# rishikksh20/FastSpeech2

Measured on AMD Instinct MI355X. Metric: mel-frames/sec, higher is better.
Workload: dtype bf16x3 (FFN conv: f16 x f16 + block-scaled e4m3 cross terms; the decoder's: block-scaled e2m1 cross terms, one E8M0 scale per 16-channel block on both operands); 1 GPU; c3: batch=64 LJSpeech-shape; default.yaml dims, free-running, random-init weights (seed 0), duration bias calibrated to 7.87 frames/phoneme; precision=mix_mx4, utterances=64, phonemes=4528, parallelism=single GPU, launch=eager, device-driven layout (no host sync), overlap_encoder=False, streams=3

## Files before the change

fastspeech2_amd/csrc/elementwise.h:

```cpp
#pragma once
#include "common.h"

namespace fs2 {

__global__ void build_row_meta(const int* start, const int* len, int B, int rpad, int* row_pos, int* row_seq) {
    const int row = blockIdx.x * blockDim.x + threadIdx.x;
    if (row >= rpad) return;
    int lo = 0, hi = B;
    while (lo < hi) {
        const int mid = (lo + hi) >> 1;
        if (start[mid] <= row) lo = mid + 1; else hi = mid;
    }
    const int b = lo - 1;
    int pos = -1, seq = -1;
    if (b >= 0 && row - start[b] < len[b]) { pos = row - start[b]; seq = b; }
    row_pos[row] = pos;
    row_seq[row] = seq;
}

__global__ __launch_bounds__(1024) void frame_layout_dev(const int* olens, int B, int compat, int masked, int row_cap, int work_cap,
                                                         int lmax_cap, int pe_rows, int* start, int* len, int* klen, int* vlen,
                                                         int* rank_tmp, int* woff_tmp, int* pcum, int2* work, int* dims, int* status = nullptr, int gap = 8) {
    constexpr int kStage = 4096;
    __shared__ int s_len[kStage], s_vlen[kStage], s_order[kStage];
// ... 195 lines not shown
        }
        if (lane == 63) wsum[wave] = x;
        __syncthreads();
        int off = carry_s;
        for (int w = 0; w < wave; ++w) off += wsum[w];
        if (t < T) cum[(size_t)b * Tmax + t] = off + x;
        __syncthreads();
        if (tid == 255) carry_s = off + x;
        __syncthreads();
    }
    if (tid == 0) {
        const int tt = bad_s ? -1 : (ones ? T : total);
        if (olens) olens[b] = tt;
        if (olens32) olens32[b] = tt;
    }
}

__global__ __launch_bounds__(256) void lr_expand(const float* hs, int D, const int* tok_start, const int* ilen,
                                                 const int* cum, int Tmax, const int* row_pos, const int* row_seq,
                                                 int uniform_len, const int* vlen, int R, float* out,
                                                 int* index_rows, void* planes = nullptr) {
    const int row = __builtin_amdgcn_readfirstlane(blockIdx.x * 4 + (threadIdx.x >> 6));
    const int lane = threadIdx.x & 63;
    if (row >= R) return;
    int b, j;
    if (row_seq) { b = row_seq[row]; j = row_pos[row]; } else { b = row / uniform_len; j = row - b * uniform_len; }
    float* dst = out + (size_t)row * D;
    int idx = -1;
    if (b >= 0 && j < vlen[b]) {
        const int* c = cum + (size_t)b * Tmax;
// ... 59 lines not shown
    const float* te = Te + (size_t)qe * D;
    const float* tp = Tp + (size_t)qp * D;
    for (int c = lane * 4; c < D; c += 256) {
        float4 v = *reinterpret_cast<const float4*>(dst + c);
        const float4 a = *reinterpret_cast<const float4*>(tp + c);
        const float4 g = *reinterpret_cast<const float4*>(te + c);
        v.x = (v.x + a.x) + g.x;
        v.y = (v.y + a.y) + g.y;
        v.z = (v.z + a.z) + g.z;
        v.w = (v.w + a.w) + g.w;
        *reinterpret_cast<float4*>(dst + c) = v;
        if (planes) store_planes4(planes, row, D / 32, c, f32x4{v.x, v.y, v.z, v.w});
    }
}

template <typename T>
__global__ void unpack_rows(const T* src, int W, const int* start, const int* limit, int B, int Lout, T* dst, T fill) {
    const int64_t i = (int64_t)blockIdx.x * blockDim.x + threadIdx.x;
    const int64_t total = (int64_t)B * Lout * W;
    if (i >= total) return;
    const int w = (int)(i % W);
    const int64_t bj = i / W;
    const int j = (int)(bj % Lout), b = (int)(bj / Lout);
    dst[i] = (j < limit[b]) ? src[(size_t)(start[b] + j) * W + w] : fill;
}

__global__ void unpack_rows4(const float* src, int W4, const int* start, const int* limit, int B, int Lout, float* dst, const int* ovf = nullptr) {
    const int64_t i = (int64_t)blockIdx.x * blockDim.x + threadIdx.x;
    if (i >= (int64_t)B * Lout * W4) return;
    const int w = (int)(i % W4);
// ... 90 lines not shown
```

fastspeech2_amd/csrc/fs2_runtime.hip:

```cpp
#include <hip/hip_runtime.h>
#include <dlfcn.h>

#include <algorithm>
#include <cmath>
#include <cstdarg>
#include <cstdio>
#include <cstring>
#include <fstream>
#include <iterator>
#include <map>
#include <string>
#include <type_traits>
#include <vector>

#include "../../include/fs2.h"
#include "attn_bf16.h"
#include "attn_w32.h"
#include "attn_f32.h"
#include "common.h"
#include "elementwise.h"
#include "gemm_bf16.h"
#include "gemm_plan.h"
#include "gemm_planes.h"
#include "gemm_row4.h"
// ... 7 lines not shown
namespace {

std::string g_create_error;

struct Gemm {
    float* w = nullptr;
    void* wb = nullptr;
    void* wf = nullptr;
    void* wm = nullptr;
    int kw = 0;
    void* wm4 = nullptr;
    unsigned char* ws4 = nullptr;
    float* bias = nullptr;
    int N = 0, C = 0, Cpad = 0, ktaps = 1;
};
struct Layer {
    Gemm qkv, out, w1, w2;
    Gemm cat_x, cat_a;
    float *ln1g = nullptr, *ln1b = nullptr, *ln2g = nullptr, *ln2b = nullptr;
    int ka = 0;
    int kh = 0;
};
struct Predictor {
    std::vector<Gemm> conv;
    std::vector<float*> lng, lnb;
    float *lin_w = nullptr, *lin_b = nullptr;
};
struct FusedPredictors {
    bool ok = false;
    Gemm c0, c1;
// ... 87 lines not shown
        if (sf.gcount() > 0) sh.update(blk.data(), (size_t)sf.gcount());
    }
    return sh.hex16() == want;
}
bool audit_clean() {
    static const bool ok = audit_clean_of_this_binary();
    return ok;
}

Options& opts() {
    static Options o = [] {
        Options x;
        x.bm = env_int("FS2_BM", -1); x.row8 = env_int("FS2_ROW8", -1); x.qkv8 = env_int("FS2_QKV8", -1);
        x.nosplitk = env_int("FS2_NOSPLITK", 0) != 0; x.f32_rows = env_int("FS2_F32_ROWS", 0) != 0; x.mt8 = env_int("FS2_MT8", -1); x.qkv_split = env_int("FS2_QKV_SPLIT", -1); x.op_att_planes = env_int("FS2_OP_ATT_PLANES", 0); x.fuse_var = env_int("FS2_FUSE_VAR", 1); x.bal = env_int("FS2_BAL", 0); x.w32 = env_int("FS2_ATTN_W32", -1);
        x.row4 = env_int("FS2_ROW4", -1); x.mt4 = env_int("FS2_MT4", -1); x.ffn2_mx = env_int("FS2_FFN2_MX", 1); x.qkv4 = env_int("FS2_QKV4", -1); x.post_mx = env_int("FS2_POST_MX", 1);
        if (!audit_clean()) {
            x.w32 = 0; x.row4 = 0; x.qkv4 = 0;
            fprintf(stderr, "libfs2_hip: no clean ISA-audit record of this binary (libfs2_hip.audit.json next to it): attn_w32 and gemm_row4_bf16 are switched "
                            "off, attn_bf16 / gemm_row8_bf16 run instead; rebuild with `python -c 'import __graft_entry__ as g; g.build()'`\n");
        }
        return x;
    }();
    return o;
}

inline int padded_head_dim(int dk) { return dk <= 64 ? 64 : (dk <= 128 ? 128 : (dk <= 192 ? 192 : (dk <= 256 ? 256 : 0))); }
inline int att_width(int D, int heads) { return heads * padded_head_dim(D / heads); }

inline int base_precision(int p) { return (p == FS2_PREC_MIX_F16X2 || p == FS2_PREC_MIX_F16X1 || p == FS2_PREC_MIX_MX || p == FS2_PREC_MIX_MX4) ? FS2_PREC_BF16X3 : p; }
constexpr int kFfnMx = 9;
// ... 66 lines not shown
struct ProfRec { std::string name; hipEvent_t e0, e1; double flops, bytes; };

}

struct fs2_handle {
    fs2_config cfg;
    std::string err;
    bool loaded = false;
    std::vector<void*> allocs;
    float* enc_embed = nullptr;
    Stack enc, dec;
    Predictor dur, energy, pitch;
    FusedPredictors var2;
    float *ebins = nullptr, *pbins = nullptr, *Te = nullptr, *Tp = nullptr;
    Gemm dec_in; float *dec_in_lng = nullptr, *dec_in_lnb = nullptr;
    Gemm feat;
    std::vector<Gemm> post;
    bool encoded = false;
    HostLayout tok;
    DevLayout dtok;
    float* enc_final = nullptr;
    int* cum = nullptr;
    int* o32 = nullptr;
    int enc_B = 0, enc_Tmax = 0, enc_compat = 0;
    long enc_ntok = 0;
    float* kp = nullptr; size_t kp_cap = 0;
    int cur_regime = 0;
    int* counters = nullptr;
    int* cur_status = nullptr;
    int gap = kGap;
    void* enc_ws = nullptr;
    std::vector<void*> graph_pinned;
    bool prof = false;
    std::string prof_filter;
    std::vector<ProfRec> recs;
};
// ... 595 lines not shown
        a.relu_pre = 1; a.ln_g = p.lng[l]; a.ln_b = p.lnb[l]; a.ln_eps = 1e-12f;
        if (last) { a.dot_w = p.lin_w; a.dot_b = p.lin_b; a.dot_out = out_rows; }
        a.scratch = out;
        a.Xp = Xp; a.xp_scratch = xps;
        if (xps && !last) { a.Yp = xps; a.yp_chunks = round_up(p.conv[l].N, 32) / 32; }
        if (xps && !last) Xp = xps; else Xp = nullptr;
        snprintf(nm, sizeof nm, "%s.conv%d", tag, (int)l);
        int rc = launch_gemm(h, s, nm, a, prec);
        if (rc) return rc;
        in = out; ld = p.conv[l].N;
    }
    return FS2_OK;
}

int run_predictors_fused(fs2_handle* h, hipStream_t s, const FusedPredictors& v, const float* X, int ldx, int R, const int* row_pos, const int* Rp,
                         const void* Xp, void* xps, float* vp, float* vs, float* e_rows, float* p_rows, int prec) {
    const int chans = v.c0.N / 2;
    int rc;
    const bool row8 = row_regime(h->cur_regime ? h->cur_regime : R, opts().row8);
    if (row8 && (chans == 256 || chans == 384)) {
        const Predictor* ps[2] = {&h->energy, &h->pitch};
        for (int g = 0; g < 2; ++g) {
            GemmArgs a = gemm_args(ps[g]->conv[0], X, ldx, R, row_pos, nullptr, chans);
            a.Rp = Rp; a.relu_pre = 1; a.ln_g = ps[g]->lng[0]; a.ln_b = ps[g]->lnb[0]; a.ln_eps = 1e-12f;
            a.Xp = Xp; a.xp_scratch = xps; a.Yp = vp; a.yp_chunks = v.c0.N / 32; a.yp_col_off = g * chans; a.scratch = vs;
            if ((rc = launch_gemm(h, s, g ? "pitch.conv0" : "energy.conv0", a, prec))) return rc;
        }
    } else {
        GemmArgs a = gemm_args(v.c0, X, ldx, R, row_pos, nullptr, v.c0.N);
        a.Rp = Rp; a.relu_pre = 1; a.ln_g = v.ln0g; a.ln_b = v.ln0b; a.ln_eps = 1e-12f; a.ln_groups = 2;
        a.Xp = Xp; a.xp_scratch = xps; a.Yp = vp; a.yp_chunks = v.c0.N / 32; a.scratch = vs;
        if ((rc = launch_gemm(h, s, "var.conv0", a, prec))) return rc;
    }
    GemmArgs a = gemm_args(v.c1, nullptr, v.c0.N, R, row_pos, nullptr, v.c1.N);
    a.Rp = Rp; a.relu_pre = 1; a.ln_g = v.ln1g; a.ln_b = v.ln1b; a.ln_eps = 1e-12f; a.ln_groups = 2; a.k_groups = 2;
// ... 239 lines not shown
    st.alpha = scaled ? L.copy(pe_pre + ".alpha", {}) : nullptr;
}

void load_predictor(Loader& L, Predictor& p, const std::string& pre, int nlayers, int idim, int chans, int k) {
    p.conv.clear(); p.lng.clear(); p.lnb.clear();
    for (int l = 0; l < nlayers; ++l) {
        const std::string c = pre + ".conv." + std::to_string(l);
        p.conv.push_back(L.gemm({c + ".0.weight"}, {c + ".0.bias"}, chans, l == 0 ? idim : chans, k, false));
        p.lng.push_back(L.copy(c + ".2.layer_norm.weight", {chans}));
        p.lnb.push_back(L.copy(c + ".2.layer_norm.bias", {chans}));
    }
    p.lin_w = L.copy(pre + ".linear.weight", {1, chans});
    p.lin_b = L.copy(pre + ".linear.bias", {1});
}

void free_weights(fs2_handle* h) {
    for (void* p : h->allocs) hipFree(p);
    h->allocs.clear();
    h->loaded = false;
}

int check_batch(fs2_handle* h, const fs2_batch& b) {
    if (b.B <= 0 || b.Tmax <= 0 || !b.ilens) return fail(h, FS2_ERR_ARG, "batch: B=%d Tmax=%d ilens=%p", b.B, b.Tmax, (const void*)b.ilens);
    for (int i = 0; i < b.B; ++i)
        if (b.ilens[i] <= 0 || b.ilens[i] > b.Tmax) return fail(h, FS2_ERR_ARG, "ilens[%d]=%lld outside [1,%d]", i, (long long)b.ilens[i], b.Tmax);
    if (b.precision < FS2_PREC_FP32 || b.precision > FS2_PREC_MIX_MX4) return fail(h, FS2_ERR_ARG, "unknown precision mode %d", b.precision);
    if (b.regime_tokens < 0 || b.regime_utterances < 0 || (b.regime_tokens > 0) != (b.regime_utterances > 0))
        return fail(h, FS2_ERR_ARG, "batch: regime_tokens=%lld / regime_utterances=%d must be given together (0 / 0 = this call's own batch)", (long long)b.regime_tokens, b.regime_utterances);
    return FS2_OK;
}
// ... 11 lines not shown

void token_layout(const fs2_batch& b, HostLayout& L, int gap) {
    std::vector<int> len(b.B), klen(b.B), vlen(b.B);
    for (int i = 0; i < b.B; ++i) {
        vlen[i] = klen[i] = (int)b.ilens[i];
        len[i] = b.compat_padded ? b.Tmax : (int)b.ilens[i];
    }
    build_layout(L, b.B, len, klen, vlen, gap);
}

struct TokenPlan {
    size_t total;
};

size_t carve_tokens(const fs2_config& c, const fs2_batch& b, const HostLayout& L, void* ws, size_t cap, int** meta, StackBufs* sb,
                    float** p0, float** p1, float** dlog_rows, int64_t** dint, int** cum, int** olens32, bool* ok, float** kp = nullptr, size_t* kp_cap = nullptr) {
    Bump bp(ws, cap);
    const size_t R = L.Rpad;
    int* m = bp.take<int>(layout_dev_ints(L));
    float* x0 = bp.take<float>(R * c.adim);
    float* x1 = bp.take<float>(R * c.adim);
    const size_t eDp = att_width(c.adim, c.aheads);
    float* qkv = bp.take<float>(R * 3 * eDp);
    float* ctx = bp.take<float>(R * eDp);
    float* hid = bp.take<float>(R * (size_t)round_up(c.eunits, 32));
    __bf16* qkh = bp.take<__bf16>(R * 2 * eDp);
    __bf16* qkl = bp.take<__bf16>(R * 2 * eDp);
    __bf16* vth = bp.take<__bf16>(R * eDp);
    __bf16* vtl = bp.take<__bf16>(R * eDp);
    const size_t pw = round_up(c.adim, 32);
    float* x0p = bp.take<float>(R * pw);
    float* x1p = bp.take<float>(R * pw);
    float* xps = bp.take<float>(R * (size_t)round_up(std::max(c.adim, c.dur_chans), 32));
    float* q0 = bp.take<float>(R * c.dur_chans);
    float* q1 = bp.take<float>(R * c.dur_chans);
    float* dl = bp.take<float>(R);
    int64_t* di = bp.take<int64_t>((size_t)b.B * b.Tmax);
    int* cu = bp.take<int>((size_t)b.B * b.Tmax);
    int* o32 = bp.take<int>(b.B);
    const size_t kcap = (size_t)4 * std::min<size_t>(R, kSplitRows) * 1024;
    float* kpb = bp.take<float>(kcap);
    if (kp) *kp = kpb;
    if (kp_cap) *kp_cap = kcap;
    if (meta) *meta = m;
    if (sb) { sb->x0 = x0; sb->x1 = x1; sb->qkv = qkv; sb->ctx = ctx; sb->hid = hid; sb->qkh = qkh; sb->qkl = qkl; sb->vth = vth; sb->vtl = vtl; sb->x0p = x0p; sb->x1p = x1p; sb->xps = xps; }
    if (p0) *p0 = q0;
    if (p1) *p1 = q1;
    if (dlog_rows) *dlog_rows = dl;
    if (dint) *dint = di;
    if (cum) *cum = cu;
    if (olens32) *olens32 = o32;
    if (ok) *ok = bp.ok();
    return align_up(bp.off, 256);
}

struct FrameBufs {
// ... 190 lines not shown
    h->Tp = L.dalloc((size_t)c.n_bins * c.adim);
    {
        const fs2_tensor_desc *we = L.get("energy_embed.weight", {c.adim, c.n_bins}), *be = L.get("energy_embed.bias", {c.adim});
        const fs2_tensor_desc *wp = L.get("pitch_embed.weight", {c.adim, c.n_bins}), *bp = L.get("pitch_embed.bias", {c.adim});
        if (we && be && wp && bp && h->Te && h->Tp) {
            const int tot = c.adim * c.n_bins;
            hipLaunchKernelGGL(onehot_table, dim3((tot + 255) / 256), dim3(256), 0, s, (const float*)we->data, (const float*)be->data, c.adim, c.n_bins, h->Te);
            hipLaunchKernelGGL(onehot_table, dim3((tot + 255) / 256), dim3(256), 0, s, (const float*)wp->data, (const float*)bp->data, c.adim, c.n_bins, h->Tp);
        }
    }
    if (c.decoder_input_layer) {
        h->dec_in = L.gemm({"decoder.embed.0.weight"}, {"decoder.embed.0.bias"}, c.ddim, c.adim, 1, true);
        h->dec_in_lng = L.copy("decoder.embed.1.weight", {c.ddim});
        h->dec_in_lnb = L.copy("decoder.embed.1.bias", {c.ddim});
    }
    h->feat = L.gemm({"feat_out.weight"}, {"feat_out.bias"}, c.odim * std::max(c.reduction_factor, 1), c.ddim, 1, true);
    h->post.clear();
    for (int l = 0; l < c.postnet_layers; ++l) {
        const std::string p = "postnet.postnet." + std::to_string(l);
        const int ic = (l == 0) ? c.odim : c.postnet_chans;
        const int oc = (l == c.postnet_layers - 1) ? c.odim : c.postnet_chans;
        h->post.push_back(L.gemm({p + ".0.weight"}, {}, oc, ic, c.postnet_filts, false, c.use_batch_norm ? p + ".1" : std::string()));
    }
    if (L.rc) { free_weights(h); return L.rc; }
    HIP_TRY(h, hipGetLastError());
    HIP_TRY(h, hipStreamSynchronize(s));
    h->loaded = true;
    return FS2_OK;
}

// ... 42 lines not shown
    int rc = check_batch(h, io->batch);
    if (rc) return rc;
    if (!io->xs || !io->olens || !io->workspace) return fail(h, FS2_ERR_ARG, "fs2_encode: xs/olens/workspace must be given");
    if (io->duration_alpha < 0.f) return fail(h, FS2_ERR_ARG, "fs2_encode: duration_alpha %g must be > 0 (0 = 1.0)", (double)io->duration_alpha);
    DeviceGuard g(h->cfg.device);
    HIP_TRY(h, g.err);
    hipStream_t s = (hipStream_t)stream;
    const fs2_config& c = h->cfg;
    const fs2_batch& b = io->batch;
    const int prec = base_precision(b.precision), ffn_terms = ffn_f16_terms(b.precision);
    h->encoded = false;
    token_layout(b, h->tok, h->gap);
    const HostLayout& L = h->tok;
    if (L.len.size() && *std::max_element(L.len.begin(), L.len.end()) > h->enc.pe_rows)
        return fail(h, FS2_ERR_ARG, "sequence longer than the positional table (%d rows): extend `pe` and reload", h->enc.pe_rows);
    int* meta; StackBufs sb; float *p0, *p1, *dlog_rows; int64_t* dint; int* cum; int* o32; bool ok;
    carve_tokens(c, b, L, io->workspace, io->workspace_bytes, &meta, &sb, &p0, &p1, &dlog_rows, &dint, &cum, &o32, &ok, &h->kp, &h->kp_cap);
    if (!ok) return fail(h, FS2_ERR_WORKSPACE, "fs2_encode: workspace too small");
    const int tok_regime = regime_rows_of(b, true);
    h->cur_regime = tok_regime; h->cur_status = nullptr;
    if ((rc = upload_layout(h, s, L, meta, h->dtok))) return rc;
    const DevLayout& dl = h->dtok;
    const bool enc_pl = prec != FS2_PREC_FP32;
    {
        Scope sc(h, s, "enc.embed", 0, 4.0 * L.R * c.adim * 2);
        hipLaunchKernelGGL(embed_pe, dim3((L.R + 3) / 4), dim3(256), 0, s, io->xs, b.Tmax, h->enc_embed, c.idim, c.adim, h->enc.pe,
                           h->enc.alpha, c.use_scaled_pos_enc ? 1.0f : sqrtf((float)c.adim), dl.row_pos, dl.row_seq, L.R, sb.x0,
                           enc_pl && c.adim % 32 == 0 ? sb.x0p : nullptr);
        HIP_TRY(h, hipGetLastError());
    }
    if ((rc = run_stack(h, s, "enc", h->enc, c.adim, c.aheads, L.R, L, dl, 1, sb, prec, enc_pl && c.adim % 32 == 0, true, tok_regime, ffn_terms))) return rc;
    if ((rc = run_predictor(h, s, "dur", h->dur, sb.x0, c.adim, L.R, dl.row_pos, p0, p1, dlog_rows, prec, enc_pl ? sb.x0p : nullptr, sb.xps))) return rc;
    {
        Scope sc(h, s, "dur.post", 0, 0);
        const int n = b.B * b.Tmax;
        hipLaunchKernelGGL(dur_finalize, dim3((n + 255) / 256), dim3(256), 0, s, dlog_rows, dl.start, dl.vlen, b.B, b.Tmax, io->d_log, dint, io->d_int);
        HIP_TRY(h, hipGetLastError());
        hipLaunchKernelGGL(dur_scan, dim3(b.B), dim3(256), 0, s, io->ds ? io->ds : dint, b.Tmax, dl.vlen, cum, io->olens, o32,
                           io->duration_alpha > 0.f ? io->duration_alpha : 1.f, io->xs, c.idim);
        HIP_TRY(h, hipGetLastError());
    }
    if (io->enc_out) {
        if ((rc = unpack<float>(h, s, sb.x0, c.adim, dl.start, dl.vlen, b.B, b.Tmax, io->enc_out, 0.f))) return rc;
    }
    h->enc_final = sb.x0; h->cum = cum; h->o32 = o32; h->enc_B = b.B; h->enc_Tmax = b.Tmax; h->enc_compat = b.compat_padded;
    h->enc_ntok = 0;
    for (int i = 0; i < b.B; ++i) h->enc_ntok += (long)b.ilens[i];
    h->enc_ws = io->workspace;
    h->encoded = true;
    return FS2_OK;
}

size_t fs2_frame_workspace_bytes(const fs2_handle* h, const fs2_batch* b, const int64_t* olens) {
    if (!h || !b || !olens || b->B <= 0) return 0;
    HostLayout L;
    frame_layout(*b, olens, 0, L, h->gap);
    return carve_frames(h->cfg, L, nullptr, 0, nullptr, nullptr);
}
// ... 49 lines not shown
    HostLayout L;
    if (devlay) capacity_layout(b, io->row_capacity, io->Lmax, L);
    else frame_layout(b, io->olens, io->masked, L, h->gap);
    FrameBufs f; bool ok;
    carve_frames(c, L, io->workspace, io->workspace_bytes, &f, &ok);
    if (!ok) return fail(h, FS2_ERR_WORKSPACE, "fs2_decode: workspace too small");
    h->kp = f.kp; h->kp_cap = f.kp_cap;
    DevLayout dl;
    if (devlay) {
        if ((rc = device_layout(h, s, L, f.meta, dl, h->o32, b.compat_padded, io->masked, io->Lmax, h->dec.pe_rows, io->status))) return rc;
    } else if ((rc = upload_layout(h, s, L, f.meta, dl))) return rc;
    const int R = L.R;
    const int regime_rows = regime_rows_of(b, false);
    h->cur_regime = regime_rows; h->cur_status = devlay ? io->status : nullptr;
    void* hfr_planes = (prec != FS2_PREC_FP32 && c.adim % 32 == 0) ? f.sb.x1p : nullptr;
    {
        Scope sc(h, s, "lr.expand", 0, 4.0 * R * c.adim * 2);
        hipLaunchKernelGGL(lr_expand, dim3((R + 3) / 4), dim3(256), 0, s, h->enc_final, c.adim, h->dtok.start, h->dtok.vlen, h->cum, b.Tmax,
                           dl.row_pos, dl.row_seq, 0, dl.vlen, R, f.hfr, f.lri, hfr_planes);
        HIP_TRY(h, hipGetLastError());
    }
    const bool need_e = (io->es == nullptr) || io->e_out, need_p = (io->ps == nullptr) || io->p_out;
    if (need_e && need_p && prec != FS2_PREC_FP32 && h->var2.ok && hfr_planes && opts().fuse_var) {
        if ((rc = run_predictors_fused(h, s, h->var2, f.hfr, c.adim, R, dl.row_pos, dl.dims, hfr_planes, f.sb.xps, f.vp, f.vs, f.e_rows, f.p_rows, prec))) return rc;
    } else {
        if (need_e && (rc = run_predictor(h, s, "energy", h->energy, f.hfr, c.adim, R, dl.row_pos, f.t0, f.t1, f.e_rows, prec, hfr_planes, f.sb.xps, dl.dims))) return rc;
        if (need_p && (rc = run_predictor(h, s, "pitch", h->pitch, f.hfr, c.adim, R, dl.row_pos, f.t0, f.t1, f.p_rows, prec, hfr_planes, f.sb.xps, dl.dims))) return rc;
    }
    {
        Scope sc(h, s, "var.embed", 0, 4.0 * R * c.adim * 4);
        hipLaunchKernelGGL(bucket_embed, dim3((R + 3) / 4), dim3(256), 0, s, f.hfr, c.adim, dl.row_pos, dl.row_seq, R, io->es, io->es_stride,
                           io->ps, io->ps_stride, f.e_rows, f.p_rows, h->ebins, h->pbins, c.n_bins - 1, h->Te, h->Tp, f.qe, f.qp, hfr_planes);
        HIP_TRY(h, hipGetLastError());
    }
    const bool dec_pl = prec != FS2_PREC_FP32;
    const bool po = dec_pl && planes_only_regime(h, prec, R, regime_rows) && (ffn_terms == 0 || ffn_terms == kFfnMx || ffn_terms == kFfnMx4);
    if (c.decoder_input_layer) {
        GemmArgs a = gemm_args(h->dec_in, f.hfr, c.adim, R, dl.row_pos, po ? nullptr : f.sb.x0, c.ddim);
        a.Rp = dl.dims; a.regime_rows = regime_rows;
        a.ln_g = h->dec_in_lng; a.ln_b = h->dec_in_lnb; a.ln_eps = 1e-5f; a.act_post = 1;
        a.pe = h->dec.pe; a.pe_ld = c.ddim; a.pe_alpha = h->dec.alpha; a.x_scale = c.use_scaled_pos_enc ? 1.f : sqrtf((float)c.ddim);
        a.Xp = hfr_planes; a.xp_scratch = f.sb.xps;
        if (dec_pl) { a.Yp = f.sb.x0p; a.yp_chunks = c.ddim / 32; }
        if ((rc = launch_gemm(h, s, "dec.in", a, prec))) return rc;
    } else {
        Scope sc(h, s, "dec.in.pe", 0.0, 8.0 * R * c.ddim);
        HIP_TRY(h, hipMemcpyAsync(f.sb.x0, f.hfr, (size_t)R * c.ddim * sizeof(float), hipMemcpyDeviceToDevice, s));
        GemmArgs a;
        memset(&a, 0, sizeof a);
        a.N = c.ddim; a.R = R; a.row_pos = dl.row_pos; a.Y = f.sb.x0; a.ldy = c.ddim;
        a.pe = h->dec.pe; a.pe_ld = c.ddim; a.pe_alpha = h->dec.alpha; a.x_scale = c.use_scaled_pos_enc ? 1.f : sqrtf((float)c.ddim);
        if (dec_pl) { a.Yp = f.sb.x0p; a.yp_chunks = c.ddim / 32; }
// ... 305 lines not shown
    else if (n == "FS2_ROW8") o.row8 = value;
    else if (n == "FS2_QKV8") o.qkv8 = value;
    else if (n == "FS2_NOSPLITK") o.nosplitk = value > 0;
    else if (n == "FS2_F32_ROWS") o.f32_rows = value > 0;
    else if (n == "FS2_MT8") o.mt8 = value;
    else if (n == "FS2_QKV_SPLIT") o.qkv_split = value;
    else if (n == "FS2_OP_ATT_PLANES") o.op_att_planes = value;
    else if (n == "FS2_FUSE_VAR") o.fuse_var = value != 0;
    else if (n == "FS2_BAL") o.bal = value < 0 ? 0 : value;
    else if (n == "FS2_ATTN_W32") o.w32 = value;
    else if (n == "FS2_ROW4") o.row4 = value;
    else if (n == "FS2_MT4") o.mt4 = value;
    else if (n == "FS2_FFN2_MX") o.ffn2_mx = value != 0;
    else if (n == "FS2_QKV4") o.qkv4 = value;
    else if (n == "FS2_POST_MX") o.post_mx = value != 0;
    else return fail(nullptr, FS2_ERR_ARG, "fs2_set_option: unknown option %s", name);
    return FS2_OK;
}

int fs2_get_option(const char* name, int32_t* value) {
    if (!name || !value) return fail(nullptr, FS2_ERR_ARG, "fs2_get_option: null argument");
    const Options& o = opts();
    const std::string n = name;
    if (n == "FS2_AUDIT_CLEAN") *value = audit_clean() ? 1 : 0;
    else if (n == "attn_w32_active") *value = o.w32 != 0;
    else if (n == "row4_active") *value = o.row4 != 0;
    else if (n == "qkv4_active") *value = o.qkv4 != 0 && o.row4 != 0;
    else if (n == "FS2_BM") *value = o.bm;
    else if (n == "FS2_ROW8") *value = o.row8;
    else if (n == "FS2_QKV8") *value = o.qkv8;
    else if (n == "FS2_NOSPLITK") *value = o.nosplitk;
    else if (n == "FS2_F32_ROWS") *value = o.f32_rows;
    else if (n == "FS2_MT8") *value = o.mt8;
    else if (n == "FS2_QKV_SPLIT") *value = o.qkv_split;
    else if (n == "FS2_OP_ATT_PLANES") *value = o.op_att_planes;
    else if (n == "FS2_FUSE_VAR") *value = o.fuse_var;
    else if (n == "FS2_BAL") *value = o.bal;
    else if (n == "FS2_ATTN_W32") *value = o.w32;
    else if (n == "FS2_ROW4") *value = o.row4;
    else if (n == "FS2_MT4") *value = o.mt4;
    else if (n == "FS2_FFN2_MX") *value = o.ffn2_mx;
    else if (n == "FS2_QKV4") *value = o.qkv4;
    else if (n == "FS2_POST_MX") *value = o.post_mx;
    else return fail(nullptr, FS2_ERR_ARG, "fs2_get_option: unknown option %s", name);
    return FS2_OK;
}

int fs2_get_counter(fs2_handle* h, void* stream, const char* name, int64_t* value, int32_t reset) {
    if (!h || !name || !value) return fail(h, FS2_ERR_ARG, "fs2_get_counter: null argument");
    if (std::string(name) != "attn_slow_path_waves") return fail(h, FS2_ERR_ARG, "fs2_get_counter: unknown counter %s", name);
    DeviceGuard g(h->cfg.device);
    HIP_TRY(h, g.err);
    hipStream_t s = (hipStream_t)stream;
    int v = 0;
    HIP_TRY(h, hipMemcpyAsync(&v, h->counters, sizeof(int), hipMemcpyDeviceToHost, s));
    if (reset) HIP_TRY(h, hipMemsetAsync(h->counters, 0, sizeof(int), s));
    HIP_TRY(h, hipStreamSynchronize(s));
    *value = v;
// ... 114 lines not shown
```

fastspeech2_amd/csrc/gemm_plan.h:

```cpp
#pragma once
#include <algorithm>

#include "gemm_args.h"

namespace fs2 {

constexpr int kPlanErrArg = -1, kPlanErrHip = -2, kPlanErrState = -3, kPlanErrUnsupported = -6;
constexpr int kPlanFp32 = 0, kPlanBf16x3 = 1;
constexpr int kPlanMaxHalo = 16;
constexpr int kPlanBN = 128;

struct Options {
    int bm = -1;
    int bal = 0;
    int row8 = -1;
    int qkv8 = -1;
    int nosplitk = 0;
    int f32_rows = 0;
    int fuse_var = 1;
    int mt8 = -1;
    int op_att_planes = 0;
    int qkv_split = -1;
    int w32 = -1;
    int row4 = -1;
    int mt4 = -1;
    int qkv4 = -1;
    int ffn2_mx = 1;
    int post_mx = 1;
};

constexpr int kSplitRegime = 8192, kSplitRows = 16384;
constexpr int kCus = 256;

inline bool row_regime(long regime_rows, int forced) { return forced >= 0 ? forced != 0 : (regime_rows + 127) / 128 >= 128; }

inline long rows_in_use(const GemmArgs& a, long rows) { return a.regime_rows > 0 ? std::min<long>(rows, a.regime_rows) : rows; }

inline int row8_mt(long rows) {
    const long t128 = (rows + 127) / 128, t192 = (rows + 191) / 192;
    return (t128 > kCus && t192 <= kCus) ? 3 : 2;
}

inline int row4_mt(long rows) {
// ... 215 lines not shown
```

Before: 9.998 million mel-frames/s.

## Project encoder tokens before length regulation; gather per-frame projections for predictors and decoder input

The first variance-predictor conv (split into taps) and the decoder input linear are moved from frame rows to token rows. A single stacked GEMM runs on the encoder output, and frames then gather and sum the projected token rows. The gather kernels fuse bias, ReLU and LayerNorm for the first predictor conv. For the decoder input they add pitch and energy embeddings that were pre-projected through the decoder input weight at load time, then apply LayerNorm, ReLU and positional encoding. This cuts GEMM work by roughly the frames-per-phoneme ratio and removes the lr_expand and bucket_embed passes. In exchange it adds a workspace buffer and changes the rounding order, since the bias on the pre-projected embedding tables is handled separately.

```diff
diff --git a/fastspeech2_amd/csrc/elementwise.h b/fastspeech2_amd/csrc/elementwise.h
--- a/fastspeech2_amd/csrc/elementwise.h
+++ b/fastspeech2_amd/csrc/elementwise.h
@@ -233,6 +233,23 @@
         if (olens) olens[b] = tt;
         if (olens32) olens32[b] = tt;
     }
+}
+
+__device__ __forceinline__ int lr_token_index(int b, int j, const int* cum, int Tmax, const int* ilen, const int* vlen) {
+    if (b < 0 || j < 0 || j >= vlen[b]) return -1;
+    const int* c = cum + (size_t)b * Tmax;
+    int lo = 0, hi = ilen[b];
+    while (lo < hi) {
+        const int mid = (lo + hi) >> 1;
+        if (c[mid] <= j) lo = mid + 1; else hi = mid;
+    }
+    return lo;
+}
+
+__global__ void lr_index_only(const int* cum, int Tmax, const int* ilen, const int* row_pos, const int* row_seq, const int* vlen, int R, int* index_rows) {
+    const int row = blockIdx.x * blockDim.x + threadIdx.x;
+    if (row >= R) return;
+    index_rows[row] = lr_token_index(row_seq[row], row_pos[row], cum, Tmax, ilen, vlen);
 }
 
 __global__ __launch_bounds__(256) void lr_expand(const float* hs, int D, const int* tok_start, const int* ilen,
@@ -322,6 +339,163 @@
     }
 }
 
+struct TokGatherArgs {
+    const float* P; int ldp;
+    const int* tok_start;
+    const int* lri;
+    const int *row_pos, *row_seq;
+    int R;
+    int chans;
+    const float *bias, *ln_g, *ln_b;
+    void* vp;
+    int col0, D;
+    const float *es, *ps; int es_stride, ps_stride;
+    const float *e_rows, *p_rows;
+    const float *ebins, *pbins; int nb;
+    const float *TE, *TP;
+    int *qe_rows, *qp_rows;
+    const float *ln_g2, *ln_b2;
+    const float* pe; const float* pe_alpha; float x_scale;
+    float* x0; void* x0p;
+};
+
+__global__ __launch_bounds__(256) void var_gather0(TokGatherArgs a) {
+    const int unit = blockIdx.x * 4 + (threadIdx.x >> 6);
+    const int row = unit >> 1, grp = unit & 1;
+    const int lane = threadIdx.x & 63;
+    if (row >= a.R) return;
+    const int N = a.chans, co = grp * N, nch = 2 * N / 32;
+    if (a.row_pos[row] < 0) {
+        for (int c = lane * 4; c < N; c += 256) store_planes4(a.vp, row, nch, co + c, f32x4{0.f, 0.f, 0.f, 0.f});
+        return;
+    }
+    const int t0 = a.tok_start[a.row_seq[row]];
+    const float* src[3];
+#pragma unroll
+    for (int d = 0; d < 3; ++d) {
+        const int r = row + d - 1;
+        const int tk = (r >= 0 && r < a.R) ? a.lri[r] : -1;
+        src[d] = tk >= 0 ? a.P + (size_t)(t0 + tk) * a.ldp + d * 2 * N + co : nullptr;
+    }
+    float4 v[4];
+    float s = 0.f;
+#pragma unroll
+    for (int j = 0; j < 4; ++j) {
+        const int c = lane * 4 + j * 256;
+        v[j] = make_float4(0.f, 0.f, 0.f, 0.f);
+        if (c < N) {
+#pragma unroll
+            for (int d = 0; d < 3; ++d)
+                if (src[d]) {
+                    const float4 q = *reinterpret_cast<const float4*>(src[d] + c);
+                    v[j].x += q.x; v[j].y += q.y; v[j].z += q.z; v[j].w += q.w;
+                }
+            const float4 b = *reinterpret_cast<const float4*>(a.bias + co + c);
+            v[j].x = fmaxf(v[j].x + b.x, 0.f); v[j].y = fmaxf(v[j].y + b.y, 0.f); v[j].z = fmaxf(v[j].z + b.z, 0.f); v[j].w = fmaxf(v[j].w + b.w, 0.f);
+        }
+        s += (v[j].x + v[j].y) + (v[j].z + v[j].w);
+    }
+    for (int o = 32; o > 0; o >>= 1) s += __shfl_xor(s, o);
+    const float mean = s / (float)N;
+    float q = 0.f;
+#pragma unroll
+    for (int j = 0; j < 4; ++j) {
+        const int c = lane * 4 + j * 256;
+        if (c < N) {
+            const float dx = v[j].x - mean, dy = v[j].y - mean, dz = v[j].z - mean, dw = v[j].w - mean;
+            q += (dx * dx + dy * dy) + (dz * dz + dw * dw);
+        }
+    }
+    for (int o = 32; o > 0; o >>= 1) q += __shfl_xor(q, o);
+    const float rstd = 1.f / sqrtf(q / (float)N + 1e-12f);
+#pragma unroll
+    for (int j = 0; j < 4; ++j) {
+        const int c = lane * 4 + j * 256;
+        if (c < N) {
+            const float4 g = *reinterpret_cast<const float4*>(a.ln_g + co + c);
+            const float4 b = *reinterpret_cast<const float4*>(a.ln_b + co + c);
+            store_planes4(a.vp, row, nch, co + c, f32x4{(v[j].x - mean) * rstd * g.x + b.x, (v[j].y - mean) * rstd * g.y + b.y,
+                                                      (v[j].z - mean) * rstd * g.z + b.z, (v[j].w - mean) * rstd * g.w + b.w});
+        }
+    }
+}
+
+__global__ __launch_bounds__(256) void dec_in_gather(TokGatherArgs a) {
+    const int row = __builtin_amdgcn_readfirstlane(blockIdx.x * 4 + (threadIdx.x >> 6));
+    const int lane = threadIdx.x & 63;
+    if (row >= a.R) return;
+    const int D = a.D, nch = D / 32;
+    const int pos = a.row_pos[row];
+    float* y = a.x0 ? a.x0 + (size_t)row * D : nullptr;
+    if (pos < 0) {
+        if (lane == 0) { if (a.qe_rows) a.qe_rows[row] = -1; if (a.qp_rows) a.qp_rows[row] = -1; }
+        for (int c = lane * 4; c < D; c += 256) {
+            if (y) *reinterpret_cast<float4*>(y + c) = make_float4(0.f, 0.f, 0.f, 0.f);
+            store_planes4(a.x0p, row, nch, c, f32x4{0.f, 0.f, 0.f, 0.f});
+        }
+        return;
+    }
+    const int b = a.row_seq[row];
+    const float e = a.es ? (pos < a.es_stride ? a.es[(size_t)b * a.es_stride + pos] : 0.f) : a.e_rows[row];
+    const float p = a.ps ? (pos < a.ps_stride ? a.ps[(size_t)b * a.ps_stride + pos] : 0.f) : a.p_rows[row];
+    const int qe = bucket_index(e, a.ebins, a.nb);
+    const int qp = bucket_index(p, a.pbins, a.nb);
+    if (lane == 0) { if (a.qe_rows) a.qe_rows[row] = qe; if (a.qp_rows) a.qp_rows[row] = qp; }
+    const int tk = a.lri[row];
+    const float* ph = tk >= 0 ? a.P + (size_t)(a.tok_start[b] + tk) * a.ldp + a.col0 : nullptr;
+    const float* te = a.TE + (size_t)qe * D;
+    const float* tp = a.TP + (size_t)qp * D;
+    float4 v[4];
+    float s = 0.f;
+#pragma unroll
+    for (int j = 0; j < 4; ++j) {
+        const int c = lane * 4 + j * 256;
+        v[j] = make_float4(0.f, 0.f, 0.f, 0.f);
+        if (c < D) {
+            if (ph) v[j] = *reinterpret_cast<const float4*>(ph + c);
+            const float4 g = *reinterpret_cast<const float4*>(tp + c);
+            const float4 h = *reinterpret_cast<const float4*>(te + c);
+            v[j].x = (v[j].x + g.x) + h.x; v[j].y = (v[j].y + g.y) + h.y; v[j].z = (v[j].z + g.z) + h.z; v[j].w = (v[j].w + g.w) + h.w;
+        }
+        s += (v[j].x + v[j].y) + (v[j].z + v[j].w);
+    }
+    for (int o = 32; o > 0; o >>= 1) s += __shfl_xor(s, o);
+    const float mean = s / (float)D;
+    float q = 0.f;
+#pragma unroll
+    for (int j = 0; j < 4; ++j) {
+        const int c = lane * 4 + j * 256;
+        if (c < D) {
+            const float dx = v[j].x - mean, dy = v[j].y - mean, dz = v[j].z - mean, dw = v[j].w - mean;
+            q += (dx * dx + dy * dy) + (dz * dz + dw * dw);
+        }
+    }
+    for (int o = 32; o > 0; o >>= 1) q += __shfl_xor(q, o);
+    const float rstd = 1.f / sqrtf(q / (float)D + 1e-5f);
+    const float alpha = a.pe_alpha ? a.pe_alpha[0] : 1.f;
+#pragma unroll
+    for (int j = 0; j < 4; ++j) {
+        const int c = lane * 4 + j * 256;
+        if (c < D) {
+            const float4 g = *reinterpret_cast<const float4*>(a.ln_g2 + c);
+            const float4 bt = *reinterpret_cast<const float4*>(a.ln_b2 + c);
+            const float4 pv = *reinterpret_cast<const float4*>(a.pe + (size_t)pos * D + c);
+            float4 t;
+            t.x = fmaxf((v[j].x - mean) * rstd * g.x + bt.x, 0.f) * a.x_scale + alpha * pv.x;
+            t.y = fmaxf((v[j].y - mean) * rstd * g.y + bt.y, 0.f) * a.x_scale + alpha * pv.y;
+            t.z = fmaxf((v[j].z - mean) * rstd * g.z + bt.z, 0.f) * a.x_scale + alpha * pv.z;
+            t.w = fmaxf((v[j].w - mean) * rstd * g.w + bt.w, 0.f) * a.x_scale + alpha * pv.w;
+            if (y) *reinterpret_cast<float4*>(y + c) = t;
+            store_planes4(a.x0p, row, nch, c, f32x4{t.x, t.y, t.z, t.w});
+        }
+    }
+}
+
+__global__ void conv_tap_rows(const float* w, int N, int C, int k, int tap, float* out) {
+    const int i = blockIdx.x * blockDim.x + threadIdx.x;
+    if (i < N * C) out[i] = w[(size_t)i * k + tap];
+}
+
 template <typename T>
 __global__ void unpack_rows(const T* src, int W, const int* start, const int* limit, int B, int Lout, T* dst, T fill) {
     const int64_t i = (int64_t)blockIdx.x * blockDim.x + threadIdx.x;
diff --git a/fastspeech2_amd/csrc/fs2_runtime.hip b/fastspeech2_amd/csrc/fs2_runtime.hip
--- a/fastspeech2_amd/csrc/fs2_runtime.hip
+++ b/fastspeech2_amd/csrc/fs2_runtime.hip
@@ -45,6 +45,14 @@
     float* bias = nullptr;
     int N = 0, C = 0, Cpad = 0, ktaps = 1;
 };
+inline Gemm gemm_rows_from(const Gemm& g, int n0) {
+    Gemm r;
+    r.N = g.N - n0; r.C = g.C; r.Cpad = g.Cpad; r.ktaps = g.ktaps;
+    r.w = g.w + (size_t)n0 * g.ktaps * g.Cpad;
+    r.wb = reinterpret_cast<__bf16*>(g.wb) + (size_t)n0 * (g.Cpad / 32) * g.ktaps * 64;
+    r.bias = g.bias ? g.bias + n0 : nullptr;
+    return r;
+}
 struct Layer {
     Gemm qkv, out, w1, w2;
     Gemm cat_x, cat_a;
@@ -162,6 +170,7 @@
         x.bm = env_int("FS2_BM", -1); x.row8 = env_int("FS2_ROW8", -1); x.qkv8 = env_int("FS2_QKV8", -1);
         x.nosplitk = env_int("FS2_NOSPLITK", 0) != 0; x.f32_rows = env_int("FS2_F32_ROWS", 0) != 0; x.mt8 = env_int("FS2_MT8", -1); x.qkv_split = env_int("FS2_QKV_SPLIT", -1); x.op_att_planes = env_int("FS2_OP_ATT_PLANES", 0); x.fuse_var = env_int("FS2_FUSE_VAR", 1); x.bal = env_int("FS2_BAL", 0); x.w32 = env_int("FS2_ATTN_W32", -1);
         x.row4 = env_int("FS2_ROW4", -1); x.mt4 = env_int("FS2_MT4", -1); x.ffn2_mx = env_int("FS2_FFN2_MX", 1); x.qkv4 = env_int("FS2_QKV4", -1); x.post_mx = env_int("FS2_POST_MX", 1);
+        x.tokproj = env_int("FS2_TOKPROJ", 3) & 3; x.tokproj_f32 = env_int("FS2_TOKPROJ_F32", 0) != 0;
         if (!audit_clean()) {
             x.w32 = 0; x.row4 = 0; x.qkv4 = 0;
             fprintf(stderr, "libfs2_hip: no clean ISA-audit record of this binary (libfs2_hip.audit.json next to it): attn_w32 and gemm_row4_bf16 are switched "
@@ -258,12 +267,15 @@
     FusedPredictors var2;
     float *ebins = nullptr, *pbins = nullptr, *Te = nullptr, *Tp = nullptr;
     Gemm dec_in; float *dec_in_lng = nullptr, *dec_in_lnb = nullptr;
+    Gemm tokw; float *TEd = nullptr, *TPd = nullptr;
     Gemm feat;
     std::vector<Gemm> post;
     bool encoded = false;
     HostLayout tok;
     DevLayout dtok;
     float* enc_final = nullptr;
+    float* tokP = nullptr;
+    bool tokP_conv = false;
     int* cum = nullptr;
     int* o32 = nullptr;
     int enc_B = 0, enc_Tmax = 0, enc_compat = 0;
@@ -889,11 +901,16 @@
 }
 
 int run_predictors_fused(fs2_handle* h, hipStream_t s, const FusedPredictors& v, const float* X, int ldx, int R, const int* row_pos, const int* Rp,
-                         const void* Xp, void* xps, float* vp, float* vs, float* e_rows, float* p_rows, int prec) {
+                         const void* Xp, void* xps, float* vp, float* vs, float* e_rows, float* p_rows, int prec, const TokGatherArgs* tg = nullptr) {
     const int chans = v.c0.N / 2;
     int rc;
     const bool row8 = row_regime(h->cur_regime ? h->cur_regime : R, opts().row8);
-    if (row8 && (chans == 256 || chans == 384)) {
+    if (tg) {
+        Scope sc(h, s, "var.gather0", 0.0, 4.0 * R * chans * (6.0 + 2.0));
+        hipLaunchKernelGGL(var_gather0, dim3((2 * (size_t)R + 3) / 4), dim3(256), 0, s, *tg);
+        hipError_t e = hipGetLastError();
+        if (e != hipSuccess) return fail(h, FS2_ERR_HIP, "var.gather0 launch: %s", hipGetErrorString(e));
+    } else if (row8 && (chans == 256 || chans == 384)) {
         const Predictor* ps[2] = {&h->energy, &h->pitch};
         for (int g = 0; g < 2; ++g) {
             GemmArgs a = gemm_args(ps[g]->conv[0], X, ldx, R, row_pos, nullptr, chans);
@@ -1163,6 +1180,43 @@
     p.lin_b = L.copy(pre + ".linear.bias", {1});
 }
 
+inline int tok_proj_cols(const fs2_config& c) {
+    const bool ok = c.decoder_input_layer && c.var_kernel == 3 && c.var_layers == 2 && c.var_chans % 128 == 0 && c.var_chans <= 1024 && c.adim % 32 == 0 &&
+                    c.ddim % 32 == 0 && c.ddim <= 1024;
+    return ok ? 6 * c.var_chans + c.ddim : 0;
+}
+
+void load_tok_proj(Loader& L, fs2_handle* h) {
+    const fs2_config& c = h->cfg;
+    hipStream_t s = L.s;
+    const int ch = c.var_chans, Nt = tok_proj_cols(c);
+    const fs2_tensor_desc* wsrc[2] = {L.get("energy_predictor.predictor.conv.0.0.weight", {ch, c.adim, 3}), L.get("pitch_predictor.predictor.conv.0.0.weight", {ch, c.adim, 3})};
+    const fs2_tensor_desc* win = L.get("decoder.embed.0.weight", {c.ddim, c.adim});
+    if (!wsrc[0] || !wsrc[1] || !win) return;
+    float* stk = nullptr;
+    if (hipMalloc((void**)&stk, (size_t)Nt * c.adim * sizeof(float)) != hipSuccess) { if (!L.rc) L.rc = fail(h, FS2_ERR_HIP, "hipMalloc failed"); return; }
+    L.synth_mem.push_back(stk);
+    for (int tap = 0; tap < 3; ++tap)
+        for (int g = 0; g < 2; ++g)
+            hipLaunchKernelGGL(conv_tap_rows, dim3((ch * c.adim + 255) / 256), dim3(256), 0, s, (const float*)wsrc[g]->data, ch, c.adim, 3, tap, stk + (size_t)(tap * 2 + g) * ch * c.adim);
+    hipMemcpyAsync(stk + (size_t)6 * ch * c.adim, win->data, (size_t)c.ddim * c.adim * sizeof(float), hipMemcpyDeviceToDevice, s);
+    auto* nd = new fs2_tensor_desc(*win);
+    auto* nn = new std::string("tok_proj#stack");
+    nd->name = nn->c_str(); nd->data = stk; nd->ndim = 2; nd->shape[0] = Nt; nd->shape[1] = c.adim;
+    L.synth.push_back(nd); L.synth_names.push_back(nn);
+    L.m[*nn] = nd;
+    h->tokw = L.gemm({*nn}, {}, Nt, c.adim, 1, true);
+    h->TPd = L.dalloc((size_t)c.n_bins * c.ddim);
+    h->TEd = L.dalloc((size_t)c.n_bins * c.ddim);
+    if (L.rc || !h->TPd || !h->TEd || !h->Te || !h->Tp) { h->tokw = Gemm(); return; }
+    for (int t = 0; t < 2; ++t) {
+        GemmArgs a = gemm_args(h->dec_in, t ? h->Te : h->Tp, c.adim, c.n_bins, nullptr, t ? h->TEd : h->TPd, c.ddim);
+        if (t) a.bias = nullptr;
+        const int rc = launch_gemm(nullptr, s, t ? "load.TEd" : "load.TPd", a, FS2_PREC_FP32);
+        if (rc && !L.rc) L.rc = fail(h, rc, "%s", g_create_error.c_str());
+    }
+}
+
 void free_weights(fs2_handle* h) {
     for (void* p : h->allocs) hipFree(p);
     h->allocs.clear();
@@ -1204,7 +1258,7 @@
 };
 
 size_t carve_tokens(const fs2_config& c, const fs2_batch& b, const HostLayout& L, void* ws, size_t cap, int** meta, StackBufs* sb,
-                    float** p0, float** p1, float** dlog_rows, int64_t** dint, int** cum, int** olens32, bool* ok, float** kp = nullptr, size_t* kp_cap = nullptr) {
+                    float** p0, float** p1, float** dlog_rows, int64_t** dint, int** cum, int** olens32, bool* ok, float** kp = nullptr, size_t* kp_cap = nullptr, float** tokp = nullptr) {
     Bump bp(ws, cap);
     const size_t R = L.Rpad;
     int* m = bp.take<int>(layout_dev_ints(L));
@@ -1230,6 +1284,8 @@
     int* o32 = bp.take<int>(b.B);
     const size_t kcap = (size_t)4 * std::min<size_t>(R, kSplitRows) * 1024;
     float* kpb = bp.take<float>(kcap);
+    float* tkp = (tok_proj_cols(c) && b.precision != FS2_PREC_FP32) ? bp.take<float>(R * (size_t)tok_proj_cols(c)) : nullptr;
+    if (tokp) *tokp = tkp;
     if (kp) *kp = kpb;
     if (kp_cap) *kp_cap = kcap;
     if (meta) *meta = m;
@@ -1450,6 +1506,8 @@
         h->dec_in_lng = L.copy("decoder.embed.1.weight", {c.ddim});
         h->dec_in_lnb = L.copy("decoder.embed.1.bias", {c.ddim});
     }
+    h->tokw = Gemm(); h->TEd = h->TPd = nullptr; h->tokP = nullptr;
+    if (tok_proj_cols(c) && h->var2.ok && !L.rc) load_tok_proj(L, h);
     h->feat = L.gemm({"feat_out.weight"}, {"feat_out.bias"}, c.odim * std::max(c.reduction_factor, 1), c.ddim, 1, true);
     h->post.clear();
     for (int l = 0; l < c.postnet_layers; ++l) {
@@ -1522,8 +1580,8 @@
     const HostLayout& L = h->tok;
     if (L.len.size() && *std::max_element(L.len.begin(), L.len.end()) > h->enc.pe_rows)
         return fail(h, FS2_ERR_ARG, "sequence longer than the positional table (%d rows): extend `pe` and reload", h->enc.pe_rows);
-    int* meta; StackBufs sb; float *p0, *p1, *dlog_rows; int64_t* dint; int* cum; int* o32; bool ok;
-    carve_tokens(c, b, L, io->workspace, io->workspace_bytes, &meta, &sb, &p0, &p1, &dlog_rows, &dint, &cum, &o32, &ok, &h->kp, &h->kp_cap);
+    int* meta; StackBufs sb; float *p0, *p1, *dlog_rows, *tokp; int64_t* dint; int* cum; int* o32; bool ok;
+    carve_tokens(c, b, L, io->workspace, io->workspace_bytes, &meta, &sb, &p0, &p1, &dlog_rows, &dint, &cum, &o32, &ok, &h->kp, &h->kp_cap, &tokp);
     if (!ok) return fail(h, FS2_ERR_WORKSPACE, "fs2_encode: workspace too small");
     const int tok_regime = regime_rows_of(b, true);
     h->cur_regime = tok_regime; h->cur_status = nullptr;
@@ -1550,6 +1608,17 @@
     }
     if (io->enc_out) {
         if ((rc = unpack<float>(h, s, sb.x0, c.adim, dl.start, dl.vlen, b.B, b.Tmax, io->enc_out, 0.f))) return rc;
+    }
+    h->tokP = nullptr; h->tokP_conv = false;
+    if (enc_pl && h->tokw.N && tokp && opts().tokproj) {
+        const bool conv = (opts().tokproj & 1) && opts().fuse_var;
+        const int n0 = conv ? 0 : 6 * c.var_chans;
+        const Gemm g = gemm_rows_from(h->tokw, n0);
+        GemmArgs a = gemm_args(g, sb.x0, c.adim, L.R, dl.row_pos, tokp + n0, h->tokw.N);
+        a.Xp = sb.x0p; a.xp_scratch = sb.xps;
+        a.kpart = h->kp; a.kpart_cap = 0;
+        if ((rc = launch_gemm(h, s, "tok.proj", a, opts().tokproj_f32 ? FS2_PREC_FP32 : prec))) return rc;
+        h->tokP = tokp; h->tokP_conv = conv;
     }
     h->enc_final = sb.x0; h->cum = cum; h->o32 = o32; h->enc_B = b.B; h->enc_Tmax = b.Tmax; h->enc_compat = b.compat_padded;
     h->enc_ntok = 0;
@@ -1629,20 +1698,30 @@
     const int regime_rows = regime_rows_of(b, false);
     h->cur_regime = regime_rows; h->cur_status = devlay ? io->status : nullptr;
     void* hfr_planes = (prec != FS2_PREC_FP32 && c.adim % 32 == 0) ? f.sb.x1p : nullptr;
-    {
+    const bool need_e = (io->es == nullptr) || io->e_out, need_p = (io->ps == nullptr) || io->p_out;
+    const bool fused_var = need_e && need_p && prec != FS2_PREC_FP32 && h->var2.ok && hfr_planes && opts().fuse_var;
+    const int tokproj = (prec != FS2_PREC_FP32 && h->tokP && c.decoder_input_layer) ? (opts().tokproj & ((fused_var && h->tokP_conv) ? 3 : 2)) : 0;
+    TokGatherArgs tg;
+    memset(&tg, 0, sizeof tg);
+    tg.P = h->tokP; tg.ldp = h->tokw.N; tg.tok_start = h->dtok.start; tg.lri = f.lri; tg.row_pos = dl.row_pos; tg.row_seq = dl.row_seq; tg.R = R;
+    tg.chans = c.var_chans; tg.bias = h->var2.c0.bias; tg.ln_g = h->var2.ln0g; tg.ln_b = h->var2.ln0b; tg.vp = f.vp;
+    if (tokproj == 3) {
+        Scope sc(h, s, "lr.index", 0, 4.0 * R);
+        hipLaunchKernelGGL(lr_index_only, dim3((R + 255) / 256), dim3(256), 0, s, h->cum, b.Tmax, h->dtok.vlen, dl.row_pos, dl.row_seq, dl.vlen, R, f.lri);
+        HIP_TRY(h, hipGetLastError());
+    } else {
         Scope sc(h, s, "lr.expand", 0, 4.0 * R * c.adim * 2);
         hipLaunchKernelGGL(lr_expand, dim3((R + 3) / 4), dim3(256), 0, s, h->enc_final, c.adim, h->dtok.start, h->dtok.vlen, h->cum, b.Tmax,
                            dl.row_pos, dl.row_seq, 0, dl.vlen, R, f.hfr, f.lri, hfr_planes);
         HIP_TRY(h, hipGetLastError());
     }
-    const bool need_e = (io->es == nullptr) || io->e_out, need_p = (io->ps == nullptr) || io->p_out;
-    if (need_e && need_p && prec != FS2_PREC_FP32 && h->var2.ok && hfr_planes && opts().fuse_var) {
-        if ((rc = run_predictors_fused(h, s, h->var2, f.hfr, c.adim, R, dl.row_pos, dl.dims, hfr_planes, f.sb.xps, f.vp, f.vs, f.e_rows, f.p_rows, prec))) return rc;
+    if (fused_var) {
+        if ((rc = run_predictors_fused(h, s, h->var2, f.hfr, c.adim, R, dl.row_pos, dl.dims, hfr_planes, f.sb.xps, f.vp, f.vs, f.e_rows, f.p_rows, prec, (tokproj & 1) ? &tg : nullptr))) return rc;
     } else {
         if (need_e && (rc = run_predictor(h, s, "energy", h->energy, f.hfr, c.adim, R, dl.row_pos, f.t0, f.t1, f.e_rows, prec, hfr_planes, f.sb.xps, dl.dims))) return rc;
         if (need_p && (rc = run_predictor(h, s, "pitch", h->pitch, f.hfr, c.adim, R, dl.row_pos, f.t0, f.t1, f.p_rows, prec, hfr_planes, f.sb.xps, dl.dims))) return rc;
     }
-    {
+    if (!(tokproj & 2)) {
         Scope sc(h, s, "var.embed", 0, 4.0 * R * c.adim * 4);
         hipLaunchKernelGGL(bucket_embed, dim3((R + 3) / 4), dim3(256), 0, s, f.hfr, c.adim, dl.row_pos, dl.row_seq, R, io->es, io->es_stride,
                            io->ps, io->ps_stride, f.e_rows, f.p_rows, h->ebins, h->pbins, c.n_bins - 1, h->Te, h->Tp, f.qe, f.qp, hfr_planes);
@@ -1650,7 +1729,16 @@
     }
     const bool dec_pl = prec != FS2_PREC_FP32;
     const bool po = dec_pl && planes_only_regime(h, prec, R, regime_rows) && (ffn_terms == 0 || ffn_terms == kFfnMx || ffn_terms == kFfnMx4);
-    if (c.decoder_input_layer) {
+    if (tokproj & 2) {
+        tg.col0 = 6 * c.var_chans; tg.D = c.ddim; tg.es = io->es; tg.ps = io->ps; tg.es_stride = io->es_stride; tg.ps_stride = io->ps_stride;
+        tg.e_rows = f.e_rows; tg.p_rows = f.p_rows; tg.ebins = h->ebins; tg.pbins = h->pbins; tg.nb = c.n_bins - 1; tg.TE = h->TEd; tg.TP = h->TPd;
+        tg.qe_rows = f.qe; tg.qp_rows = f.qp; tg.ln_g2 = h->dec_in_lng; tg.ln_b2 = h->dec_in_lnb;
+        tg.pe = h->dec.pe; tg.pe_alpha = h->dec.alpha; tg.x_scale = c.use_scaled_pos_enc ? 1.f : sqrtf((float)c.ddim);
+        tg.x0 = po ? nullptr : f.sb.x0; tg.x0p = f.sb.x0p;
+        Scope sc(h, s, "dec.in.gather", 0, 4.0 * R * c.ddim * (po ? 2.0 : 3.0));
+        hipLaunchKernelGGL(dec_in_gather, dim3((R + 3) / 4), dim3(256), 0, s, tg);
+        HIP_TRY(h, hipGetLastError());
+    } else if (c.decoder_input_layer) {
         GemmArgs a = gemm_args(h->dec_in, f.hfr, c.adim, R, dl.row_pos, po ? nullptr : f.sb.x0, c.ddim);
         a.Rp = dl.dims; a.regime_rows = regime_rows;
         a.ln_g = h->dec_in_lng; a.ln_b = h->dec_in_lnb; a.ln_eps = 1e-5f; a.act_post = 1;
@@ -1986,6 +2074,8 @@
     else if (n == "FS2_FFN2_MX") o.ffn2_mx = value != 0;
     else if (n == "FS2_QKV4") o.qkv4 = value;
     else if (n == "FS2_POST_MX") o.post_mx = value != 0;
+    else if (n == "FS2_TOKPROJ") o.tokproj = value < 0 ? 3 : (value & 3);
+    else if (n == "FS2_TOKPROJ_F32") o.tokproj_f32 = value > 0;
     else return fail(nullptr, FS2_ERR_ARG, "fs2_set_option: unknown option %s", name);
     return FS2_OK;
 }
@@ -2014,6 +2104,8 @@
     else if (n == "FS2_FFN2_MX") *value = o.ffn2_mx;
     else if (n == "FS2_QKV4") *value = o.qkv4;
     else if (n == "FS2_POST_MX") *value = o.post_mx;
+    else if (n == "FS2_TOKPROJ") *value = o.tokproj;
+    else if (n == "FS2_TOKPROJ_F32") *value = o.tokproj_f32;
     else return fail(nullptr, FS2_ERR_ARG, "fs2_get_option: unknown option %s", name);
     return FS2_OK;
 }
diff --git a/fastspeech2_amd/csrc/gemm_plan.h b/fastspeech2_amd/csrc/gemm_plan.h
--- a/fastspeech2_amd/csrc/gemm_plan.h
+++ b/fastspeech2_amd/csrc/gemm_plan.h
@@ -27,6 +27,8 @@
     int qkv4 = -1;
     int ffn2_mx = 1;
     int post_mx = 1;
+    int tokproj = 3;
+    int tokproj_f32 = 0;
 };
 
 constexpr int kSplitRegime = 8192, kSplitRows = 16384;
```

Measured after the change: 10.14 million mel-frames/s (median of 6 runs). 1.01x the previous value.
